# ubisoft/ubisoft-laforge-msmd

Hardware: AMD Instinct MI355X
Metric: FLAME frames/sec on 4s@16kHz clips (whole job; MSMD.forward motion-coefficient frames) (higher is better)
Workload: dtype bf16; 1 GPU; configs[1]: MSMD.forward, batch=32 x 4 s clips per GPU, wav2vec2-base encoder + 8-layer motion decoder, eval-mode, synthetic closed-form weights; batch_per_gpu=32, frames_per_clip=100, parallelism=dp1 (independent clips, no collective), launch=one hipGraph replay per step (the batch sits in the captured input buffers)

## Files before the change

### ubisoft-laforge-msmd_amd/csrc/gemm.hip

```cpp
#include "common.h"
#include <atomic>
#include <utility>

struct GemmArgs {
  const void* A; const void* W; const float* bias; const void* R; void* C;
  int M, N, K;
  long lda; int rows_per_batch; long a_batch_stride; long ldw, ldc, ldr;
  int act; int vec_ok; float inv_rpb;
  long strideA, strideW, strideC, strideBias, strideR;
  int mt, nt;
  int batch_inner; long strideA2, strideW2, strideC2;
  void* Z; float p_drop; const unsigned long* rng; unsigned site;
  int xn;
  int flags;
  const float* a_stats = nullptr; int a_nt = 0; const float* w_colsum = nullptr;
  const float* r_stats = nullptr; int r_nt = 0; const float* r_gamma = nullptr; const float* r_beta = nullptr;
  float* stats_out = nullptr; float ln_eps = 1e-5f;
  int stagger_ticks = 0;
};

enum : int {
  GF_WRITE_THROUGH = 1, GF_PAIRED_STORES = 2, GF_STAGGER = 4,
  GF_ACT_BWD = 8,
  GF_ONE_TILE = 16, GF_NO_256 = 32,
  GF_W_BELOW_32 = 64,
};
struct GemmActWord { int act, hint, flags; };
static constexpr GemmActWord gemm_unpack_act(int act) {
  return {act & 0xff, (act >> 8) & 0xff, ((act >> 16) & 7) | (((act >> 19) & 7) << 4)};
}
static_assert(gemm_unpack_act(MSMD_GEMM_WRITE_THROUGH).flags == GF_WRITE_THROUGH && gemm_unpack_act(MSMD_GEMM_PAIRED_STORES).flags == GF_PAIRED_STORES &&
              gemm_unpack_act(MSMD_GEMM_STAGGER).flags == GF_STAGGER && gemm_unpack_act(MSMD_GEMM_ONE_TILE_PER_WORKGROUP).flags == GF_ONE_TILE &&
              gemm_unpack_act(MSMD_GEMM_NO_256_TILE).flags == GF_NO_256 && gemm_unpack_act(MSMD_GEMM_W_BELOW_32).flags == GF_W_BELOW_32 && gemm_unpack_act(~0).flags == (0x7f & ~GF_ACT_BWD),
              "internal flag bits follow include/msmd_hip.h; no bit of `act` sets the internal one");
enum : int {
  GV_GENERIC = 0,
  GV_SPLIT_128 = 1, GV_SPLIT_64 = 5,
  GV_64_DEEP = 9, GV_64 = 12,
  GV_256x64 = 14,
  GV_192 = 15,
  GV_128 = 17,
  GV_128_AB = 13, GV_128_ONE_AB = 66,
  GV_256 = 80,
};

enum GemmEpi : int { EPI_ALL = 0, EPI_PLAIN = 1, EPI_LN_OPERAND = 2, EPI_LN_RESIDUAL = 3 };
constexpr int ACT_RUNTIME = -1;
constexpr int epia(GemmEpi e, int act) { return e + 10 * (1 + act); }
constexpr GemmEpi epia_family(int code) { return (GemmEpi)(code % 10); }
constexpr int epia_act(int code) { return code / 10 - 1; }

template <typename T> struct Mfma;
template <> struct Mfma<bf16_t> {
  static __device__ __forceinline__ void run(const u32x4& a, const u32x4& b, f32x4& acc) {
    acc = __builtin_amdgcn_mfma_f32_16x16x32_bf16(__builtin_bit_cast(bf16x8, a), __builtin_bit_cast(bf16x8, b),
                                                  acc, 0, 0, 0);
  }
};
template <> struct Mfma<f16_t> {
  static __device__ __forceinline__ void run(const u32x4& a, const u32x4& b, f32x4& acc) {
    acc = __builtin_amdgcn_mfma_f32_16x16x32_f16(__builtin_bit_cast(f16x8, a), __builtin_bit_cast(f16x8, b), acc, 0, 0, 0);
  }
};
template <> struct Mfma<float> {
  static __device__ __forceinline__ void run(const u32x4& a, const u32x4& b, f32x4& acc) {
#pragma unroll
    for (int e = 0; e < 4; ++e)
      acc = __builtin_amdgcn_mfma_f32_16x16x4f32(__uint_as_float(a[e]), __uint_as_float(b[e]), acc, 0, 0, 0);
  }
};

__device__ __forceinline__ int lds_off(int row, int chunk) { return row * 128 + ((chunk ^ ((row >> 1) & 7)) << 4); }

__device__ __forceinline__ long a_row_offset(const GemmArgs& p, int m) {
  if (p.rows_per_batch >= p.M) return (long)m * p.lda;
  int q = (int)((float)m * p.inv_rpb);
  int r = m - q * p.rows_per_batch;
  if (r < 0) { q -= 1; r += p.rows_per_batch; }
  if (r >= p.rows_per_batch) { q += 1; r -= p.rows_per_batch; }
  return (long)q * p.a_batch_stride + (long)r * p.lda;
}

template <typename TO> __device__ __forceinline__ float act_out(float x, int act) {
  if (act == MSMD_ACT_GELU) return sizeof(TO) == 2 ? gelu_poly16(x) : gelu_erf(x);
  if (act == MSMD_ACT_ELU) return elu1(x);
  return x;
}
template <typename TO, int ACT> __device__ __forceinline__ float act_out_c(float x, int act) {
  if constexpr (ACT == MSMD_ACT_GELU) return sizeof(TO) == 2 ? gelu_poly16(x) : gelu_erf(x);
  else if constexpr (ACT == MSMD_ACT_ELU) return elu1(x);
  else if constexpr (ACT == MSMD_ACT_NONE) return x;
  else return act_out<TO>(x, act);
}

__device__ __forceinline__ void store16_wt(void* p, const u32x4 v) {
  asm volatile("global_store_dwordx4 %0, %1, off sc1\n\ts_nop 1" ::"v"(p), "v"(v) : "memory");
}
__device__ __forceinline__ void store8_wt(void* p, const u32x2 v) {
  asm volatile("global_store_dwordx2 %0, %1, off sc1\n\ts_nop 1" ::"v"(p), "v"(v) : "memory");
}
template <typename TO> __device__ __forceinline__ void store4_out(TO* p, const float* v, bool wt) {
  if constexpr (sizeof(TO) == 4) {
    const f32x4 o = f32x4{v[0], v[1], v[2], v[3]};
    if (wt) store16_wt(p, __builtin_bit_cast(u32x4, o));
    else *(f32x4*)p = o;
  } else {
    const typename Vec4T<TO>::type o = pack4<TO>(v[0], v[1], v[2], v[3]);
    if (wt) store8_wt(p, __builtin_bit_cast(u32x2, o));
    else *(typename Vec4T<TO>::type*)p = o;
  }
}

template <typename TO, int FM, int FN, bool AB, bool LEAN, int ACT>
__device__ __forceinline__ void gemm_epilogue_interior(const GemmArgs& p, const f32x4 (&acc)[FN][FM], int z, int m_base,
                                                         int n_base, int fr, int fq) {
  TO* __restrict__ C = (TO*)p.C + (z / p.batch_inner) * p.strideC + (z % p.batch_inner) * p.strideC2 +
                       (long)(m_base + fr) * p.ldc + n_base + fq * 4;
  const TO* __restrict__ R = p.R ? (const TO*)p.R + z * p.strideR + (long)(m_base + fr) * p.ldr + n_base + fq * 4 : nullptr;
  const float* __restrict__ bias = p.bias ? p.bias + z * p.strideBias + n_base + fq * 4 : nullptr;
  const bool wt = p.flags & GF_WRITE_THROUGH;
  f32x4 bv[FN];
#pragma unroll
  for (int i = 0; i < FN; ++i) bv[i] = bias ? *(const f32x4*)(bias + i * 16) : f32x4{0.f, 0.f, 0.f, 0.f};
  typedef typename Vec4T<TO>::type V4;
// ... 100 lines not shown
#pragma unroll
      for (int e = 0; e < 4; ++e) v[e] = acc[i][j][e] + bv[e];
      TO* cp = C + (long)m * p.ldc + n;
      if (AB && (p.flags & GF_ACT_BWD)) {
        const TO* zp = (const TO*)p.Z + (cp - (TO*)p.C);
#pragma unroll
        for (int e = 0; e < 4; ++e)
          if (n + e < p.N) v[e] *= act_grad_fast((float)zp[e], ACT >= 0 ? ACT : p.act);
      } else {
        if (!LEAN && p.Z) {
          TO* zp = (TO*)p.Z + (cp - (TO*)p.C);
#pragma unroll
          for (int e = 0; e < 4; ++e)
            if (n + e < p.N) zp[e] = (TO)v[e];
        }
#pragma unroll
        for (int e = 0; e < 4; ++e) v[e] = act_out_c<TO, ACT>(v[e], p.act);
      }
      if (!LEAN && p.p_drop > 0.f) {
        const Philox4 rb = dropout_bits(p.rng, p.site, (unsigned long)(((long)m * p.N + n) >> 2));
        const unsigned thr = dropout_threshold(p.p_drop);
        const float c = 1.0f / (1.0f - p.p_drop);
        v[0] = rb.x >= thr ? v[0] * c : 0.f;
        v[1] = rb.y >= thr ? v[1] * c : 0.f;
        v[2] = rb.z >= thr ? v[2] * c : 0.f;
        v[3] = rb.w >= thr ? v[3] * c : 0.f;
      }
      if (p.vec_ok && n + 3 < p.N) {
        if (R) {
          const TO* rp = R + (long)m * p.ldr + n;
          if constexpr (sizeof(TO) == 4) {
            const f32x4 r = *(const f32x4*)rp;
#pragma unroll
            for (int e = 0; e < 4; ++e) v[e] += r[e];
          } else {
            const typename Vec4T<TO>::type r = *(const typename Vec4T<TO>::type*)rp;
#pragma unroll
            for (int e = 0; e < 4; ++e) v[e] += (float)r[e];
          }
        }
        store4_out<TO>(cp, v, p.flags & GF_WRITE_THROUGH);
      } else {
#pragma unroll
        for (int e = 0; e < 4; ++e) {
          if (n + e < p.N) {
            float o = v[e];
            if (R) o += to_f32(R[(long)m * p.ldr + n + e]);
            cp[e] = from_f32<TO>(o);
          }
        }
      }
    }
  }
}

template <int FM>
__device__ __forceinline__ void ln_issue(const float* stats, int nt, int M, int m_base, int fr, int fq, f32x2 (&raw)[FM][4]) {
#pragma unroll
  for (int j = 0; j < FM; ++j) {
    const f32x2* sp = (const f32x2*)stats + min(m_base + j * 16 + fr, M - 1);
#pragma unroll
    for (int q = 0; q < 4; ++q) raw[j][q] = fq + 4 * q < nt ? sp[(long)(fq + 4 * q) * M] : f32x2{0.f, 0.f};
  }
}

template <int FM>
__device__ __forceinline__ void ln_finish(const float* stats, int nt, int M, int m_base, int fr, int fq, const f32x2 (&raw)[FM][4],
                                          float inv_cols, float eps, float (&mu)[FM], float (&rs)[FM]) {
#pragma unroll
  for (int j = 0; j < FM; ++j) {
    float S = (raw[j][0][0] + raw[j][1][0]) + (raw[j][2][0] + raw[j][3][0]);
    float Q = (raw[j][0][1] + raw[j][1][1]) + (raw[j][2][1] + raw[j][3][1]);
    if (nt > 16) {
      const f32x2* sp = (const f32x2*)stats + min(m_base + j * 16 + fr, M - 1);
      for (int t = 16 + fq; t < nt; t += 4) { const f32x2 w = sp[(long)t * M]; S += w[0]; Q += w[1]; }
    }
    S += __shfl_xor(S, 16, 64); S += __shfl_xor(S, 32, 64);
    Q += __shfl_xor(Q, 16, 64); Q += __shfl_xor(Q, 32, 64);
    mu[j] = S * inv_cols;
    rs[j] = rsqrtf(fmaxf(Q * inv_cols - mu[j] * mu[j], 0.f) + eps);
  }
}

template <typename TO, int FM, int FN, int MODE, int ACT = -1>
__device__ __forceinline__ void gemm_epilogue_ln(const GemmArgs& p, const f32x4 (&acc)[FN][FM], int m_base, int n_base,
                                                 int fr, int fq, const f32x2 (&raw)[FM][4]) {
  static_assert((FN == 4 || FN == 2) && (FM >= 2 && FM <= 4), "one wave = one statistics slab of 16 FN columns, 2 to 4 fragment rows");
  constexpr int SLAB = FN * 16;
  constexpr int IB = FM == 3 ? 2 : FN;
  typedef typename Vec4T<TO>::type V4;
  const int n = n_base + fq * 4;
  float mu[FM], rs[FM];
#pragma unroll
  for (int j = 0; j < FM; ++j) { mu[j] = 0.f; rs[j] = 1.f; }
  if constexpr (MODE == 1) ln_finish<FM>(p.a_stats, p.a_nt, p.M, m_base, fr, fq, raw, 1.0f / (float)p.K, p.ln_eps, mu, rs);
  else if (p.r_stats) ln_finish<FM>(p.r_stats, p.r_nt, p.M, m_base, fr, fq, raw, 1.0f / (float)p.N, p.ln_eps, mu, rs);
  float rowS[FM], rowQ[FM], tS[FM], tQ[FM], prS[FM], prQ[FM];
#pragma unroll
  for (int j = 0; j < FM; ++j) rowS[j] = rowQ[j] = tS[j] = tQ[j] = prS[j] = prQ[j] = 0.f;
  const bool odd = fq & 1;
  const bool pair = sizeof(TO) == 2 && (p.flags & GF_PAIRED_STORES);
#pragma unroll
  for (int i0 = 0; i0 < FN; i0 += IB) {
    f32x4 bv[IB], xv[IB], yv[IB];
    V4 rr[FM][IB];
#pragma unroll
    for (int ii = 0; ii < IB; ++ii) bv[ii] = *(const f32x4*)(p.bias + n + (i0 + ii) * 16);
    if constexpr (MODE == 1) {
#pragma unroll
      for (int ii = 0; ii < IB; ++ii) xv[ii] = *(const f32x4*)(p.w_colsum + n + (i0 + ii) * 16);
    } else {
#pragma unroll
      for (int j = 0; j < FM; ++j) {
        const TO* rp = (const TO*)p.R + (long)min(m_base + j * 16 + fr, p.M - 1) * p.ldr + n;
#pragma unroll
        for (int ii = 0; ii < IB; ++ii) rr[j][ii] = *(const V4*)(rp + (i0 + ii) * 16);
      }
      if (p.r_stats) {
#pragma unroll
        for (int ii = 0; ii < IB; ++ii) { xv[ii] = *(const f32x4*)(p.r_gamma + n + (i0 + ii) * 16); yv[ii] = *(const f32x4*)(p.r_beta + n + (i0 + ii) * 16); }
      } else {
#pragma unroll
        for (int ii = 0; ii < IB; ++ii) { xv[ii] = f32x4{1.f, 1.f, 1.f, 1.f}; yv[ii] = f32x4{0.f, 0.f, 0.f, 0.f}; }
      }
    }
#pragma unroll
    for (int ii = 0; ii < IB; ++ii) {
      const int i = i0 + ii;
      V4 o[FM];
#pragma unroll
      for (int j = 0; j < FM; ++j) {
        float v[4];
#pragma unroll
        for (int e = 0; e < 4; ++e) {
          float x = acc[i][j][e];
          if constexpr (MODE == 1) x = rs[j] * (x - mu[j] * xv[ii][e]);
          v[e] = act_out_c<TO, ACT>(x + bv[ii][e], p.act);
          if constexpr (MODE == 2) v[e] += fmaf(((float)rr[j][ii][e] - mu[j]) * rs[j], xv[ii][e], yv[ii][e]);
        }
        if constexpr (sizeof(TO) == 4) o[j] = V4{v[0], v[1], v[2], v[3]};
        else o[j] = pack4<TO>(v[0], v[1], v[2], v[3]);
        if constexpr (MODE == 2) {
          float pS = 0.f, pQ = 0.f;
#pragma unroll
          for (int e = 0; e < 4; ++e) { const float w = (float)o[j][e]; pS += w; pQ = fmaf(w, w, pQ); }
          if ((i & 1) == 0) { tS[j] = pS; tQ[j] = pQ; }
          else {
            const float aS = tS[j] + pS, aQ = tQ[j] + pQ;
            if (FN == 2) { rowS[j] = aS; rowQ[j] = aQ; }
            else if ((i & 2) == 0) { prS[j] = aS; prQ[j] = aQ; }
            else { rowS[j] = prS[j] + aS; rowQ[j] = prQ[j] + aQ; }
          }
        }
      }
      bool stored = false;
      if constexpr (sizeof(TO) == 2) {
        if (pair) {
#pragma unroll
          for (int jp = 0; jp + 1 < FM; jp += 2) {
            const u32x2 a = __builtin_bit_cast(u32x2, o[jp]), b = __builtin_bit_cast(u32x2, o[jp + 1]);
            const u32x2 send = odd ? a : b;
            u32x2 recv;
            recv[0] = __shfl_xor(send[0], 16, 64);
            recv[1] = __shfl_xor(send[1], 16, 64);
            const u32x4 w = odd ? u32x4{recv[0], recv[1], b[0], b[1]} : u32x4{a[0], a[1], recv[0], recv[1]};
            const int m = m_base + jp * 16 + (odd ? 16 : 0) + fr;
            if (m < p.M) *(u32x4*)((TO*)p.C + (long)m * p.ldc + n + i * 16 - (odd ? 4 : 0)) = w;
          }
          if constexpr (FM % 2 == 1) {
            const int m2 = m_base + (FM - 1) * 16 + fr;
            if (m2 < p.M) *(V4*)((TO*)p.C + (long)m2 * p.ldc + n + i * 16) = o[FM - 1];
          }
          stored = true;
        }
      }
      if (!stored) {
#pragma unroll
        for (int j = 0; j < FM; ++j) {
          const int m = m_base + j * 16 + fr;
          if (m < p.M) *(V4*)((TO*)p.C + (long)m * p.ldc + n + i * 16) = o[j];
        }
      }
    }
  }
  if constexpr (MODE == 2) {
    if (p.stats_out) {
#pragma unroll
      for (int j = 0; j < FM; ++j) {
        rowS[j] += __shfl_xor(rowS[j], 16, 64); rowS[j] += __shfl_xor(rowS[j], 32, 64);
        rowQ[j] += __shfl_xor(rowQ[j], 16, 64); rowQ[j] += __shfl_xor(rowQ[j], 32, 64);
        const int m = m_base + j * 16 + fr;
        if (fq == 0 && m < p.M) *(f32x2*)(p.stats_out + ((long)(n_base / SLAB) * p.M + m) * 2) = f32x2{rowS[j], rowQ[j]};
      }
    }
  }
}

template <typename T, typename TO, int BM, int BN>
__global__ __launch_bounds__(256) void gemm_kernel(const GemmArgs p) {
  constexpr int E = 16 / sizeof(T);
  constexpr int BKE = 128 / sizeof(T);
  constexpr int LA = BM / 32, LW = BN / 32;
  constexpr int FM = BM / 32, FN = BN / 32;
  __shared__ __attribute__((aligned(16))) unsigned char smem[2 * (BM + BN) * 128];

  const int pid = blockIdx.x;
// ... 57 lines not shown
  const int nk = (p.K + BKE - 1) / BKE;
  load_global(0);
  store_lds(0);
  __syncthreads();
  for (int kt = 0; kt < nk; ++kt) {
    const int cur = kt & 1;
    if (kt + 1 < nk) load_global((kt + 1) * BKE);
    const unsigned char* sa = smem + cur * (BM + BN) * 128;
    const unsigned char* sw = sa + BM * 128;
#pragma unroll
    for (int g = 0; g < 2; ++g) {
      u32x4 fx[FM], fw[FN];
#pragma unroll
      for (int j = 0; j < FM; ++j) fx[j] = *(const u32x4*)(sa + lds_off(wm + j * 16 + fr, g * 4 + fq));
#pragma unroll
      for (int i = 0; i < FN; ++i) fw[i] = *(const u32x4*)(sw + lds_off(wn + i * 16 + fr, g * 4 + fq));
#pragma unroll
      for (int i = 0; i < FN; ++i)
#pragma unroll
        for (int j = 0; j < FM; ++j) Mfma<T>::run(fw[i], fx[j], acc[i][j]);
    }
    if (kt + 1 < nk) store_lds(cur ^ 1);
    __syncthreads();
  }

  gemm_epilogue<TO, FM, FN>(p, acc, z, m0 + wm, n0 + wn, fr, fq);
}

typedef __attribute__((address_space(3))) void lds_void_t;
typedef __attribute__((address_space(1))) const void gbl_void_t;

template <typename TO, int BM, int BN, int WM, int WN, int NSTAGE, bool PIPE = false, typename TI = bf16_t, int EPIA = 0>
__global__ __launch_bounds__(WM * WN * 64, (WM * WN == 8 && NSTAGE * (BM + BN) * 128 <= 80 * 1024 && (epia_family(EPIA) != EPI_ALL || BM * BN <= 128 * 128)) ? 4 : 1) void gemm2_kernel(const GemmArgs p) {
  constexpr int EPI = epia_family(EPIA), ACTK = epia_act(EPIA);
  constexpr int NW = WM * WN, NT = NW * 64;
  constexpr int STAGE = (BM + BN) * 128;
  constexpr int LPT = (BM + BN) * 8 / NT;
  constexpr int FM = BM / WM / 16, FN = BN / WN / 16;
  static_assert((BM + BN) * 8 % NT == 0, "tile chunks must divide over the threads");
  extern __shared__ __attribute__((aligned(16))) unsigned char smem[];

  const int pid = blockIdx.x;
  const int xcd = pid & 7, slot = pid >> 3;
  const int xm_n = 8 / p.xn, ntx = (p.nt + p.xn - 1) / p.xn;
  const int m_tile = (slot / ntx) * xm_n + (xcd % xm_n), n_tile = (slot % ntx) * p.xn + xcd / xm_n;
  if (m_tile >= p.mt || n_tile >= p.nt) return;
  const int z = blockIdx.z;
  const int zo = z / p.batch_inner, zi = z % p.batch_inner;
  const bf16_t* __restrict__ A = (const bf16_t*)p.A + zo * p.strideA + zi * p.strideA2;
  const bf16_t* __restrict__ W = (const bf16_t*)p.W + zo * p.strideW + zi * p.strideW2;
  const int m0 = m_tile * BM, n0 = n_tile * BN;
  const int tid = threadIdx.x, lane = tid & 63, wid = tid >> 6;

  const bf16_t* src[LPT];
#pragma unroll
  for (int i = 0; i < LPT; ++i) {
    const int id = (i * NW + wid) * 64 + lane;
    const int row = id >> 3, phys = id & 7;
    const int c = phys ^ ((row >> 1) & 7);
    if (row < BM) {
      const int m = min(m0 + row, p.M - 1);
      src[i] = A + a_row_offset(p, m) + c * 8;
    } else {
      const int n = min(n0 + row - BM, p.N - 1);
      src[i] = W + (long)n * p.ldw + c * 8;
    }
  }
  auto issue = [&](int kt, int stage) {
#pragma unroll
    for (int i = 0; i < LPT; ++i)
      __builtin_amdgcn_global_load_lds((gbl_void_t*)(src[i] + kt * 64),
                                       (lds_void_t*)(smem + stage * STAGE + (i * NW + wid) * 1024), 16, 0, 0);
  };

  const int wm = (wid / WN) * (BM / WM), wn = (wid % WN) * (BN / WN);
  const int fr = lane & 15, fq = lane >> 4;
  f32x4 acc[FN][FM];
#pragma unroll
  for (int i = 0; i < FN; ++i)
#pragma unroll
    for (int j = 0; j < FM; ++j) acc[i][j] = f32x4{0.f, 0.f, 0.f, 0.f};

  const int nk = p.K / 64;
#pragma unroll
  for (int s = 0; s < NSTAGE - 1; ++s)
    if (s < nk) issue(s, s);
  if (p.stagger_ticks > 0 && ((pid >> 8) & 1) && pid < 512) {
    const unsigned long t0 = __builtin_amdgcn_s_memrealtime();
    while ((long)(__builtin_amdgcn_s_memrealtime() - t0) < p.stagger_ticks) __builtin_amdgcn_s_sleep(16);
  }
  constexpr bool LNK = (BN == 128 || BN == 64) && WN == 2 && (FM == 2 || FM == 3) && sizeof(TO) == 2;
  constexpr bool LN_LATE = FM == 3;
  f32x2 lnraw[(LNK && !LN_LATE) ? FM : 1][4];
  if constexpr (LNK && !LN_LATE && EPI != 1) {
    if (EPI == 2 || (EPI == 0 && p.a_stats)) ln_issue<FM>(p.a_stats, p.a_nt, p.M, m0 + wm, fr, fq, lnraw);
    else if (p.r_stats) ln_issue<FM>(p.r_stats, p.r_nt, p.M, m0 + wm, fr, fq, lnraw);
  }
  int stage = 0;
  for (int kt = 0; kt < nk; ++kt) {
    if (kt + NSTAGE - 2 < nk) asm volatile("s_waitcnt vmcnt(%0)" ::"n"((NSTAGE - 2) * LPT) : "memory");
    else asm volatile("s_waitcnt vmcnt(0)" ::: "memory");
    __builtin_amdgcn_s_barrier();
    if (kt + NSTAGE - 1 < nk) issue(kt + NSTAGE - 1, (stage + NSTAGE - 1) % NSTAGE);
    const unsigned char* sa = smem + stage * STAGE;
    const unsigned char* sw = sa + BM * 128;
    if constexpr (PIPE) {
      u32x4 fx[2][FM], fw[2][FN];
#pragma unroll
      for (int g = 0; g < 2; ++g) {
#pragma unroll
        for (int j = 0; j < FM; ++j) fx[g][j] = *(const u32x4*)(sa + lds_off(wm + j * 16 + fr, g * 4 + fq));
#pragma unroll
        for (int i = 0; i < FN; ++i) fw[g][i] = *(const u32x4*)(sw + lds_off(wn + i * 16 + fr, g * 4 + fq));
      }
      __builtin_amdgcn_sched_barrier(0);
#pragma unroll
      for (int g = 0; g < 2; ++g) {
#pragma unroll
        for (int i = 0; i < FN; ++i)
#pragma unroll
          for (int j = 0; j < FM; ++j) Mfma<TI>::run(fw[g][i], fx[g][j], acc[i][j]);
        __builtin_amdgcn_sched_barrier(0);
      }
    } else {
#pragma unroll
      for (int g = 0; g < 2; ++g) {
        u32x4 fx[FM], fw[FN];
#pragma unroll
        for (int j = 0; j < FM; ++j) fx[j] = *(const u32x4*)(sa + lds_off(wm + j * 16 + fr, g * 4 + fq));
#pragma unroll
        for (int i = 0; i < FN; ++i) fw[i] = *(const u32x4*)(sw + lds_off(wn + i * 16 + fr, g * 4 + fq));
#pragma unroll
        for (int i = 0; i < FN; ++i)
#pragma unroll
          for (int j = 0; j < FM; ++j) Mfma<TI>::run(fw[i], fx[j], acc[i][j]);
      }
    }
    stage = (stage + 1 == NSTAGE) ? 0 : stage + 1;
  }
  int tid_e = tid;
  if constexpr (LN_LATE) asm volatile("" : "+v"(tid_e));
  const int wm_e = ((tid_e >> 6) / WN) * (BM / WM), wn_e = ((tid_e >> 6) % WN) * (BN / WN);
  const int fr_e = tid_e & 15, fq_e = (tid_e & 63) >> 4;
  auto run_epilogue = [&]() {
    if constexpr (EPI == 1) { gemm_epilogue<TO, FM, FN, false, true, ACTK>(p, acc, z, m0 + wm_e, n0 + wn_e, fr_e, fq_e); return; }
    if constexpr (LNK && !LN_LATE && EPI == 2) { gemm_epilogue_ln<TO, FM, FN, 1, ACTK>(p, acc, m0 + wm_e, n0 + wn_e, fr_e, fq_e, lnraw); return; }
    if constexpr (LNK && !LN_LATE && EPI == 3) { gemm_epilogue_ln<TO, FM, FN, 2, ACTK>(p, acc, m0 + wm_e, n0 + wn_e, fr_e, fq_e, lnraw); return; }
    if constexpr (LNK && LN_LATE && (EPI == 2 || EPI == 3)) {
      f32x2 late[FM][4];
      if constexpr (EPI == 2) ln_issue<FM>(p.a_stats, p.a_nt, p.M, m0 + wm_e, fr_e, fq_e, late);
      else if (p.r_stats) ln_issue<FM>(p.r_stats, p.r_nt, p.M, m0 + wm_e, fr_e, fq_e, late);
      gemm_epilogue_ln<TO, FM, FN, EPI - 1, ACTK>(p, acc, m0 + wm_e, n0 + wn_e, fr_e, fq_e, late);
      return;
    }
    if constexpr (LNK && !LN_LATE) {
      if (p.a_stats) { gemm_epilogue_ln<TO, FM, FN, 1, ACTK>(p, acc, m0 + wm_e, n0 + wn_e, fr_e, fq_e, lnraw); return; }
      if (p.r_stats || p.stats_out) { gemm_epilogue_ln<TO, FM, FN, 2, ACTK>(p, acc, m0 + wm_e, n0 + wn_e, fr_e, fq_e, lnraw); return; }
    }
    if constexpr (LNK && LN_LATE) {
      if (p.a_stats || p.r_stats || p.stats_out) {
        f32x2 late[FM][4];
        if (p.a_stats) ln_issue<FM>(p.a_stats, p.a_nt, p.M, m0 + wm_e, fr_e, fq_e, late);
        else if (p.r_stats) ln_issue<FM>(p.r_stats, p.r_nt, p.M, m0 + wm_e, fr_e, fq_e, late);
        if (p.a_stats) gemm_epilogue_ln<TO, FM, FN, 1, ACTK>(p, acc, m0 + wm_e, n0 + wn_e, fr_e, fq_e, late);
        else gemm_epilogue_ln<TO, FM, FN, 2, ACTK>(p, acc, m0 + wm_e, n0 + wn_e, fr_e, fq_e, late);
        return;
      }
    }
    gemm_epilogue<TO, FM, FN, sizeof(TO) == 2, false, ACTK>(p, acc, z, m0 + wm_e, n0 + wn_e, fr_e, fq_e);
  };
  run_epilogue();
}

template <typename TO, int BM, int BN, int WM, int WN, typename TI, int EPIA>
__global__ __launch_bounds__(WM * WN * 64, 4) void gemm2p_kernel(const GemmArgs p) {
  constexpr int EPI = epia_family(EPIA), ACTK = epia_act(EPIA);
  constexpr int NW = WM * WN, NT = NW * 64;
  constexpr int STAGE = (BM + BN) * 128;
  constexpr int LPT = (BM + BN) * 8 / NT;
  constexpr int FM = BM / WM / 16, FN = BN / WN / 16;
  static_assert(EPI >= 1 && EPI <= 3 && sizeof(TO) == 2 && NW == 8 && WN == 2 && BN == 128 && (FM == 2 || FM == 3), "the hot 8-wave tiles, inference epilogues");
  static_assert((BM + BN) * 8 % NT == 0, "tile chunks must divide over the threads");
  constexpr bool LN_LATE = FM == 3;
  extern __shared__ __attribute__((aligned(16))) unsigned char smem[];
  const int tid = threadIdx.x;
  const int xm_n = 8 / p.xn, ntx = (p.nt + p.xn - 1) / p.xn;
  const int vgrid = ((p.mt + xm_n - 1) / xm_n) * ntx * 8;
  const TI* __restrict__ A = (const TI*)p.A;
  const TI* __restrict__ W = (const TI*)p.W;
  auto next_tile = [&](int vb, int& m0, int& n0) -> int {
    for (; vb < vgrid; vb += gridDim.x) {
      const int xcd = vb & 7, slot = vb >> 3;
      const int m_tile = (slot / ntx) * xm_n + (xcd % xm_n), n_tile = (slot % ntx) * p.xn + xcd / xm_n;
      if (m_tile < p.mt && n_tile < p.nt) { m0 = m_tile * BM; n0 = n_tile * BN; return vb; }
    }
    return -1;
  };
  const TI* src[LPT];
  auto set_src = [&](int m0, int n0, int t) {
    const int lane = t & 63, wid = t >> 6;
#pragma unroll
    for (int i = 0; i < LPT; ++i) {
      const int id = (i * NW + wid) * 64 + lane;
      const int row = id >> 3, phys = id & 7;
      const int c = phys ^ ((row >> 1) & 7);
      if (row < BM) src[i] = A + a_row_offset(p, min(m0 + row, p.M - 1)) + c * 8;
      else src[i] = W + (long)min(n0 + row - BM, p.N - 1) * p.ldw + c * 8;
    }
  };
  auto issue = [&](int kt, int stage, int t) {
    const int wid = t >> 6;
#pragma unroll
    for (int i = 0; i < LPT; ++i)
      __builtin_amdgcn_global_load_lds((gbl_void_t*)(src[i] + kt * 64),
                                       (lds_void_t*)(smem + stage * STAGE + (i * NW + wid) * 1024), 16, 0, 0);
  };
  int m0 = 0, n0 = 0;
  int vb = next_tile(blockIdx.x, m0, n0);
  if (vb < 0) return;
  const int nk = p.K / 64;
  set_src(m0, n0, tid);
  int stage = 0;
  issue(0, 0, tid);
  for (;;) {
    int t_k = tid;
    asm volatile("" : "+v"(t_k));
    const int wm = ((t_k >> 6) / WN) * (BM / WM), wn = ((t_k >> 6) % WN) * (BN / WN);
    const int fr = t_k & 15, fq = (t_k & 63) >> 4;
    f32x2 lnraw[LN_LATE ? 1 : FM][4];
// ... 749 lines not shown
  if (p.Z || p.p_drop > 0.f || (p.flags & GF_ACT_BWD)) return false;
  if (((uintptr_t)p.bias & 15) || ((uintptr_t)p.C & 7) || ((uintptr_t)p.R & 7)) return false;
  if ((gemm_last_row_offset(p) + p.K) * 2 >= (1L << 32) || ((long)(p.N - 1) * p.ldw + p.K) * 2 >= (1L << 32)) return false;
  const GemmEpi epi = epia_family(gemm_epia(p, true));
  if ((p.a_stats || p.r_stats) && ((p.M & 1) || ((uintptr_t)p.a_stats & 15) || ((uintptr_t)p.r_stats & 15))) return false;
  if (epi == EPI_LN_OPERAND && (p.R || !p.bias || !p.w_colsum)) return false;
  if (epi == EPI_LN_RESIDUAL && (!p.R || !p.bias || p.act != MSMD_ACT_NONE)) return false;
  return p.act == MSMD_ACT_NONE || p.act == MSMD_ACT_GELU;
}

static bool gemm8_wins(int M, int N, int K) {
  const long tiles = (long)((M + 255) / 256) * (N / 256);
  if (tiles < 192) return false;
  const double fill = (double)tiles / (256.0 * (double)((tiles + 255) / 256));
  return fill >= 0.75 && (K >= 1024 || fill >= 0.878);
}

constexpr int GEMM8_RING = 2 * 4 * 128 * 128;
template <auto KFN, int LDS>
static int launch_gemm8(GemmArgs& p, hipStream_t st) {
  p.mt = (p.M + 255) / 256; p.nt = p.N / 256;
  const int tiles = p.mt * p.nt, cap = gemm8_workgroup_cap();
  if (tiles <= 512) p.flags |= GF_WRITE_THROUGH;
  return gemm_launch_kernel<KFN>(dim3(tiles < cap ? tiles : cap), 512, LDS, st, p);
}

static bool gemm8s_takes(const GemmArgs& p, int batch, bool split_out) {
  if (batch != 1 || p.batch_inner != 1 || (p.N % 256) || (p.K % 32) || p.K < 64 || !p.vec_ok) return false;
  if (((uintptr_t)p.bias & 15) || ((uintptr_t)p.C & 15) || ((uintptr_t)p.R & 15)) return false;
  if (split_out ? ((p.ldc % 32) || (p.R && (p.ldr % 32))) : ((p.ldc % 4) || (p.R && (p.ldr % 4)))) return false;
  if ((gemm_last_row_offset(p) + 2L * p.K) * 2 >= (1L << 32) || ((long)(p.N - 1) * p.ldw + 2L * p.K) * 2 >= (1L << 32)) return false;
  return p.act == MSMD_ACT_NONE || p.act == MSMD_ACT_GELU;
}
static bool gemm8s_wins(int M, int N, int K, bool w_below_32) {
  const long tiles = (long)((M + 255) / 256) * (N / 256);
  if (tiles < 160) return false;
  const double fill = (double)tiles / (256.0 * (double)((tiles + 255) / 256));
  return fill >= (w_below_32 ? 0.65 : 0.75);
}

template <typename TO, int BM, int BN, int WM, int WN, int NSTAGE>
static int launch_gemm2s(GemmArgs& p, int batch, hipStream_t st) {
  constexpr int lds = NSTAGE * (BM + BN) * 128;
  const dim3 grid(gemm2_xcd_grid(p, BM, BN, p.lda / 2), 1, batch);
  return dispatch_code<0, 1>((p.flags & GF_W_BELOW_32) != 0, [&](auto ws) {
    auto run = [&](auto act) {
      return gemm_launch_kernel<gemm2s_kernel<TO, BM, BN, WM, WN, NSTAGE, decltype(act)::value, decltype(ws)::value != 0>>(grid, WM * WN * 64, lds, st, p);
    };
    int r = -1;
    if constexpr (lds <= 80 * 1024) r = dispatch_code<MSMD_ACT_NONE, MSMD_ACT_GELU>(p.act, run);
    return r >= 0 ? r : run(std::integral_constant<int, ACT_RUNTIME>{});
  });
}

template <typename TO>
static int dispatch_gemm2s(GemmArgs& p, int batch, hipStream_t st, int variant) {
  switch (variant) {
    case GV_SPLIT_128: return launch_gemm2s<TO, 128, 128, 4, 2, 2>(p, batch, st);
    case GV_SPLIT_64: return launch_gemm2s<TO, 64, 64, 2, 2, 4>(p, batch, st);
    case GV_256x64: return launch_gemm2s<TO, 256, 64, 8, 1, 2>(p, batch, st);
    case GV_256:
      if (!gemm8s_takes(p, batch, sizeof(TO) == 2)) return -1;
      return dispatch_code<11, 21>(epia(EPI_PLAIN, p.act), [&](auto c) {
        return dispatch_code<0, 1>((p.flags & GF_W_BELOW_32) != 0, [&](auto ws) {
          return launch_gemm8<gemm8_kernel<f16_t, decltype(c)::value, (sizeof(TO) == 4 ? 2 : 1) + 4 * decltype(ws)::value>, GEMM8_RING>(p, st);
        });
      });
    default: return -1;
  }
}

template <typename T, typename TO>
static int launch_gemm(GemmArgs& p, int batch, hipStream_t st) {
  const bool small = (p.N <= 64) || ((long)((p.M + 127) / 128) * ((p.N + 127) / 128) * batch < 128);
  const int B = small ? 64 : 128;
  p.mt = (p.M + B - 1) / B; p.nt = (p.N + B - 1) / B;
  const dim3 grid(((p.mt + 7) / 8) * 8 * p.nt, 1, batch);
  return small ? gemm_launch_kernel<gemm_kernel<T, TO, 64, 64>>(grid, 256, 0, st, p)
               : gemm_launch_kernel<gemm_kernel<T, TO, 128, 128>>(grid, 256, 0, st, p);
}

static constexpr bool gemm2_has(int variant, bool bf16) {
  if (variant == GV_128_AB || variant == GV_128_ONE_AB) return bf16;
  return variant == GV_64_DEEP || variant == GV_64 || variant == GV_256x64 || variant == GV_192 || variant == GV_128 || variant == GV_256;
}

template <typename TO, typename TI>
static int dispatch_gemm(GemmArgs& p, int batch, hipStream_t st, int variant) {
  if (variant == GV_GENERIC) return launch_gemm<TI, TO>(p, batch, st);
  if constexpr (sizeof(TI) == 2) {
    if (!gemm2_has(variant, __is_same(TI, bf16_t))) return -1;
    if constexpr (__is_same(TI, bf16_t)) {
      if (variant == GV_128_AB) return launch_gemm2<TO, 128, 128, 4, 2, 2>(p, gemm2_xcd_grid(p, 128, 128, p.lda), batch, st);
      if (variant == GV_128_ONE_AB) return launch_gemm2<TO, 128, 128, 4, 2, 2, true>(p, gemm2_xcd_grid(p, 128, 128, p.lda), batch, st);
    }
    switch (variant) {
      case GV_64_DEEP: return launch_gemm2_epi<TO, 64, 64, 2, 2, 4, false, TI>(p, batch, st);
      case GV_64: return launch_gemm2_epi<TO, 64, 64, 2, 2, 2, false, TI>(p, batch, st);
      case GV_256x64: return launch_gemm2_epi<TO, 256, 64, 8, 1, 2, true, TI>(p, batch, st);
      case GV_192: return launch_gemm2_epi<TO, 192, 128, 4, 2, 2, true, TI>(p, batch, st);
      case GV_128: return launch_gemm2_epi<TO, 128, 128, 4, 2, 2, true, TI>(p, batch, st);
    }
    if constexpr (sizeof(TO) == 2) {
      if (!gemm8_takes(p, batch, 2)) return -1;
      return dispatch_code<11, 21, 12, 22, 13>(gemm_epia(p, true), [&](auto c) {
        constexpr int E = decltype(c)::value;
        return launch_gemm8<gemm8_kernel<TI, E>, GEMM8_RING + (epia_family(E) >= EPI_LN_OPERAND ? 8 * 4096 : 0)>(p, st);
      });
    }
  }
  return -1;
}

static bool tall_rounds_favour_192(int M, long tiles128, long tiles192) {
  if (M < 9600 || tiles192 < 256) return false;
  const double fill128 = (double)tiles128 / (512.0 * (double)((tiles128 + 511) / 512));
  const double fill192 = (double)tiles192 / (512.0 * (double)((tiles192 + 511) / 512));
  return 1.2 * fill192 > 1.03 * fill128;
}

struct GemmCall {
  const void* A = nullptr; const void* W = nullptr; const float* bias = nullptr; const void* residual = nullptr; void* C = nullptr;
  int M = 0, N = 0, K = 0, in_dtype = 0, out_dtype = 0;
  long lda = 0; int rows_per_batch = 0; long a_batch_stride = 0; long ldw = 0, ldc = 0, ldr = 0;
  int act = 0;
  int batch = 1; long strideA = 0, strideW = 0, strideC = 0, strideBias = 0, strideR = 0;
  int batch_inner = 1; long strideA2 = 0, strideW2 = 0, strideC2 = 0;
  void* z_out = nullptr; float p_drop = 0.f; const unsigned long* rng = nullptr; unsigned site = 0; int internal_flags = 0;
  const float* a_stats = nullptr; const float* w_colsum = nullptr; const float* r_stats = nullptr; const float* r_gamma = nullptr; const float* r_beta = nullptr;
  float* stats_out = nullptr; int slab_in = 0, slab_out = 0; float eps = 1e-5f;
};

static GemmArgs gemm_args(const GemmCall& c, int act, int flags, int osz, int ab = 1) {
  GemmArgs p{};
  const int rows_per_batch = c.rows_per_batch <= 0 ? c.M : c.rows_per_batch;
  p.A = c.A; p.W = c.W; p.bias = c.bias; p.R = c.residual; p.C = c.C;
  p.M = c.M; p.N = c.N; p.K = c.K;
  p.lda = ab * c.lda; p.rows_per_batch = rows_per_batch; p.a_batch_stride = ab * c.a_batch_stride;
  p.ldw = ab * c.ldw; p.ldc = c.ldc; p.ldr = c.ldr; p.act = act;
  p.inv_rpb = 1.0f / (float)rows_per_batch;
  p.strideA = ab * c.strideA; p.strideW = ab * c.strideW; p.strideC = c.strideC; p.strideBias = c.strideBias; p.strideR = c.strideR;
  p.batch_inner = c.batch_inner; p.strideA2 = ab * c.strideA2; p.strideW2 = ab * c.strideW2; p.strideC2 = c.strideC2;
  p.xn = 1;
  p.vec_ok = osz == 0 ||
             ((c.ldc % 4 == 0) && (c.strideC % 4 == 0) && (c.strideC2 % 4 == 0) && (((uintptr_t)c.C % (4 * osz)) == 0) &&
              (!c.residual || ((c.ldr % 4 == 0) && (c.strideR % 4 == 0) && (((uintptr_t)c.residual % (4 * osz)) == 0))));
  if ((flags & GF_PAIRED_STORES) && (osz != 2 || (c.ldc % 8) || (c.strideC % 8) || (c.strideC2 % 8) || ((uintptr_t)c.C % 16) || !p.vec_ok))
    flags &= ~GF_PAIRED_STORES;
  p.flags = flags;
  return p;
}

static int gemm_split_route(const GemmArgs& p, int nz, bool split_out, int hint, int flags) {
  const bool takes8 = gemm8s_takes(p, nz, split_out);
  if (hint == GV_256 && !takes8) hint = 0;
  if (hint) return (hint == GV_SPLIT_128 || hint == GV_SPLIT_64 || hint == GV_256x64 || hint == GV_256) ? hint : -1;
  if (!(flags & GF_NO_256) && (flags & GF_W_BELOW_32) && takes8 && gemm8s_wins(p.M, p.N, p.K, true)) return GV_256;
  if (p.N <= 64) return (long)((p.M + 255) / 256) * nz >= 256 ? GV_256x64 : GV_SPLIT_64;
  return (long)((p.M + 127) / 128) * ((p.N + 127) / 128) * nz >= 192 ? GV_SPLIT_128 : GV_SPLIT_64;
}

static int gemm16_route(const GemmArgs& p, int nz, int osz, bool bf16, int hint, int flags, int cols = 0) {
  const bool takes8 = (cols != 64 || !p.stats_out) && gemm8_takes(p, nz, osz);
  const bool rule8 = hint == 0 && !(flags & GF_NO_256);
  if (!(hint == GV_256 ? takes8 : !cols || (cols == 128 && (hint == GV_192 || hint == GV_128 || hint == GV_128_ONE_AB)))) hint = 0;
  if (hint) return gemm2_has(hint, bf16) ? hint : GV_GENERIC;
  const int M = p.M, N = p.N;
  const long tiles128 = (long)((M + 127) / 128) * ((N + 127) / 128) * nz;
  const long tiles192 = (long)((M + 191) / 192) * ((N + 127) / 128) * nz;
  const bool wide = cols ? cols == 128 : N > 64;
  if (rule8 && takes8 && gemm8_wins(M, N, p.K)) return GV_256;
  if (wide && M >= 16000 && tiles192 >= 400) return GV_192;
  if (wide && osz == 2 && !p.Z && !(p.p_drop > 0.f) && !(p.flags & GF_ACT_BWD) && tall_rounds_favour_192(M, tiles128, tiles192)) return GV_192;
  if (cols ? wide : wide && tiles128 >= 192) return GV_128;
  if (!cols && N <= 64 && (long)((M + 255) / 256) * nz >= 256) return GV_256x64;
  return p.K >= 1024 ? GV_64_DEEP : GV_64;
}

static int gemm_plan(GemmArgs& p, const GemmCall& c) {
  if (c.M <= 0 || c.N <= 0 || c.K <= 0 || c.batch <= 0 || c.batch_inner <= 0 || !c.A || !c.W || !c.C) return -1;
  const GemmActWord u = gemm_unpack_act(c.act);
  const int flags = u.flags | c.internal_flags, nz = c.batch * c.batch_inner;
  const auto strides_divide = [&](int E) {
    return !(c.K % E || c.lda % E || c.ldw % E || c.a_batch_stride % E || c.strideA % E || c.strideW % E || c.strideA2 % E || c.strideW2 % E);
  };
  if (c.in_dtype == MSMD_F16X2) {
    if (c.out_dtype != MSMD_F32 && c.out_dtype != MSMD_F16X2) return -1;
    if (!strides_divide(32) || c.z_out || c.p_drop != 0.f) return -1;
    if (((uintptr_t)c.A & 15) || ((uintptr_t)c.W & 15) || ((uintptr_t)c.C & 15)) return -1;
    if (c.out_dtype == MSMD_F16X2) {
      if ((c.N & 3) || c.ldc % 32 || c.strideC % 32 || c.strideC2 % 32 || (c.residual && (c.ldr % 32 || c.strideR % 32))) return -1;
      if (c.bias && (((uintptr_t)c.bias & 15) || (c.strideBias & 3))) return -1;
    }
    p = gemm_args(c, u.act, flags & (GF_WRITE_THROUGH | GF_W_BELOW_32), c.out_dtype == MSMD_F32 ? 4 : 0, 2);
    return gemm_split_route(p, nz, c.out_dtype == MSMD_F16X2, u.hint, flags);
  }
  if (c.in_dtype == MSMD_F32 ? (c.out_dtype != MSMD_F32 && c.out_dtype != MSMD_F16 && c.out_dtype != MSMD_BF16)
                             : ((c.in_dtype != MSMD_F16 && c.in_dtype != MSMD_BF16) || (c.out_dtype != c.in_dtype && c.out_dtype != MSMD_F32)))
    return -1;
  if (!strides_divide(c.in_dtype == MSMD_F32 ? 4 : 8)) return -1;
  if (((uintptr_t)c.A & 15) || ((uintptr_t)c.W & 15)) return -1;
  if (c.p_drop != 0.f && (!(c.p_drop > 0.f && c.p_drop < 1.f) || !c.rng || (c.N & 3) || c.ldc != c.N || c.batch != 1 || c.batch_inner != 1))
    return -1;
  const int osz = c.out_dtype == MSMD_F32 ? 4 : 2;
  p = gemm_args(c, u.act, flags, osz);
  p.Z = c.z_out; p.p_drop = c.p_drop; p.rng = c.rng; p.site = c.site;
  if (c.in_dtype == MSMD_F32 || (c.K % 64)) return GV_GENERIC;
  return gemm16_route(p, nz, osz, c.in_dtype == MSMD_BF16, u.hint, flags);
}

static int gemm_launch(GemmArgs& p, int in_dtype, int out_dtype, int nz, int variant, hipStream_t st) {
  switch (in_dtype * 4 + out_dtype) {
    case MSMD_F16X2 * 4 + MSMD_F32: return dispatch_gemm2s<float>(p, nz, st, variant);
    case MSMD_F16X2 * 4 + MSMD_F16X2: return dispatch_gemm2s<f16_t>(p, nz, st, variant);
    case MSMD_BF16 * 4 + MSMD_BF16: return dispatch_gemm<bf16_t, bf16_t>(p, nz, st, variant);
    case MSMD_BF16 * 4 + MSMD_F32: return dispatch_gemm<float, bf16_t>(p, nz, st, variant);
    case MSMD_F16 * 4 + MSMD_F16: return dispatch_gemm<f16_t, f16_t>(p, nz, st, variant);
    case MSMD_F16 * 4 + MSMD_F32: return dispatch_gemm<float, f16_t>(p, nz, st, variant);
    case MSMD_F32 * 4 + MSMD_F32: return dispatch_gemm<float, float>(p, nz, st, variant);
    case MSMD_F32 * 4 + MSMD_F16: return dispatch_gemm<f16_t, float>(p, nz, st, variant);
    case MSMD_F32 * 4 + MSMD_BF16: return dispatch_gemm<bf16_t, float>(p, nz, st, variant);
  }
  return -1;
}

static int gemm_run(int (*plan)(GemmArgs&, const GemmCall&), const GemmCall& c, msmd_stream_t stream) {
  GemmArgs p;
  const int variant = plan(p, c);
  const int r = variant < 0 ? -1 : gemm_launch(p, c.in_dtype, c.out_dtype, c.batch * c.batch_inner, variant, (hipStream_t)stream);
  return r >= 0 ? r : 1;
}

static GemmCall gemm_ex_call(const void* A, const void* W, const float* bias, const void* residual, void* C, int M, int N, int K, int in_dtype,
                             int out_dtype, long lda, int rows_per_batch, long a_batch_stride, long ldw, long ldc, long ldr, int act, int batch,
                             long strideA, long strideW, long strideC, long strideBias, long strideR, void* z_out, float p_drop,
                             const unsigned long* rng_state, unsigned int site) {
  GemmCall c;
  c.A = A; c.W = W; c.bias = bias; c.residual = residual; c.C = C;
  c.M = M; c.N = N; c.K = K; c.in_dtype = in_dtype; c.out_dtype = out_dtype;
  c.lda = lda; c.rows_per_batch = rows_per_batch; c.a_batch_stride = a_batch_stride; c.ldw = ldw; c.ldc = ldc; c.ldr = ldr;
  c.act = act; c.batch = batch;
  c.strideA = strideA; c.strideW = strideW; c.strideC = strideC; c.strideBias = strideBias; c.strideR = strideR;
  c.z_out = z_out; c.p_drop = p_drop; c.rng = rng_state; c.site = site;
  return c;
}

extern "C" int msmd_gemm_ex(const void* A, const void* W, const float* bias, const void* residual, void* C, int M, int N, int K, int in_dtype,
                            int out_dtype, long lda, int rows_per_batch, long a_batch_stride, long ldw, long ldc, long ldr, int act, int batch,
                            long strideA, long strideW, long strideC, long strideBias, long strideR, void* z_out, float p_drop,
                            const unsigned long* rng_state, unsigned int site, msmd_stream_t stream) {
  return gemm_run(gemm_plan, gemm_ex_call(A, W, bias, residual, C, M, N, K, in_dtype, out_dtype, lda, rows_per_batch, a_batch_stride, ldw, ldc, ldr,
                                          act, batch, strideA, strideW, strideC, strideBias, strideR, z_out, p_drop, rng_state, site), stream);
}

extern "C" int msmd_gemm(const void* A, const void* W, const float* bias, const void* residual, void* C, int M, int N, int K, int in_dtype,
                         int out_dtype, long lda, int rows_per_batch, long a_batch_stride, long ldw, long ldc, long ldr, int act, int batch,
// ... 91 lines not shown
```

Before: 829,400 frames/s.

## Add 64x128 GEMM tile variant with early-issued LayerNorm-residual epilogue operands

Adds a 64x128 tile variant (4 waves) to the generic GEMM and routes mid-size LN-column GEMMs to it when the 128x128 grid would leave most compute units idle. For the LayerNorm-residual epilogue on this tile, the residual, bias, gamma/beta and row statistics loads are issued before the K loop so their latency overlaps the main loop. The cost is extra registers held across the mainloop, which may lower occupancy.

```diff
diff --git a/ubisoft-laforge-msmd_amd/csrc/gemm.hip b/ubisoft-laforge-msmd_amd/csrc/gemm.hip
--- a/ubisoft-laforge-msmd_amd/csrc/gemm.hip
+++ b/ubisoft-laforge-msmd_amd/csrc/gemm.hip
@@ -40,6 +40,7 @@
   GV_256x64 = 14,
   GV_192 = 15,
   GV_128 = 17,
+  GV_64x128 = 18,
   GV_128_AB = 13, GV_128_ONE_AB = 66,
   GV_256 = 80,
 };
@@ -306,9 +307,31 @@
   }
 }
 
-template <typename TO, int FM, int FN, int MODE, int ACT = -1>
+template <typename TO, int FM, int FN> struct LnResOps { f32x4 bv[FN], xv[FN], yv[FN]; typename Vec4T<TO>::type rr[FM][FN]; };
+template <typename TO, int FM, int FN>
+__device__ __forceinline__ void ln_res_issue(const GemmArgs& p, int m_base, int n_base, int fr, int fq, LnResOps<TO, FM, FN>& o) {
+  typedef typename Vec4T<TO>::type V4;
+  const int n = n_base + fq * 4;
+#pragma unroll
+  for (int i = 0; i < FN; ++i) o.bv[i] = *(const f32x4*)(p.bias + n + i * 16);
+#pragma unroll
+  for (int j = 0; j < FM; ++j) {
+    const TO* rp = (const TO*)p.R + (long)min(m_base + j * 16 + fr, p.M - 1) * p.ldr + n;
+#pragma unroll
+    for (int i = 0; i < FN; ++i) o.rr[j][i] = *(const V4*)(rp + i * 16);
+  }
+  if (p.r_stats) {
+#pragma unroll
+    for (int i = 0; i < FN; ++i) { o.xv[i] = *(const f32x4*)(p.r_gamma + n + i * 16); o.yv[i] = *(const f32x4*)(p.r_beta + n + i * 16); }
+  } else {
+#pragma unroll
+    for (int i = 0; i < FN; ++i) { o.xv[i] = f32x4{1.f, 1.f, 1.f, 1.f}; o.yv[i] = f32x4{0.f, 0.f, 0.f, 0.f}; }
+  }
+}
+
+template <typename TO, int FM, int FN, int MODE, int ACT = -1, bool EARLY = false>
 __device__ __forceinline__ void gemm_epilogue_ln(const GemmArgs& p, const f32x4 (&acc)[FN][FM], int m_base, int n_base,
-                                                 int fr, int fq, const f32x2 (&raw)[FM][4]) {
+                                                 int fr, int fq, const f32x2 (&raw)[FM][4], const LnResOps<TO, FM, FN>* early = nullptr) {
   static_assert((FN == 4 || FN == 2) && (FM >= 2 && FM <= 4), "one wave = one statistics slab of 16 FN columns, 2 to 4 fragment rows");
   constexpr int SLAB = FN * 16;
   constexpr int IB = FM == 3 ? 2 : FN;
@@ -328,24 +351,34 @@
   for (int i0 = 0; i0 < FN; i0 += IB) {
     f32x4 bv[IB], xv[IB], yv[IB];
     V4 rr[FM][IB];
-#pragma unroll
-    for (int ii = 0; ii < IB; ++ii) bv[ii] = *(const f32x4*)(p.bias + n + (i0 + ii) * 16);
-    if constexpr (MODE == 1) {
-#pragma unroll
-      for (int ii = 0; ii < IB; ++ii) xv[ii] = *(const f32x4*)(p.w_colsum + n + (i0 + ii) * 16);
+    if constexpr (EARLY) {
+      static_assert(MODE == 2 && IB == FN, "the early operands are the LayerNorm-residual form's, all fragment columns at once");
+#pragma unroll
+      for (int ii = 0; ii < IB; ++ii) {
+        bv[ii] = early->bv[ii]; xv[ii] = early->xv[ii]; yv[ii] = early->yv[ii];
+#pragma unroll
+        for (int j = 0; j < FM; ++j) rr[j][ii] = early->rr[j][ii];
+      }
     } else {
 #pragma unroll
-      for (int j = 0; j < FM; ++j) {
-        const TO* rp = (const TO*)p.R + (long)min(m_base + j * 16 + fr, p.M - 1) * p.ldr + n;
-#pragma unroll
-        for (int ii = 0; ii < IB; ++ii) rr[j][ii] = *(const V4*)(rp + (i0 + ii) * 16);
-      }
-      if (p.r_stats) {
-#pragma unroll
-        for (int ii = 0; ii < IB; ++ii) { xv[ii] = *(const f32x4*)(p.r_gamma + n + (i0 + ii) * 16); yv[ii] = *(const f32x4*)(p.r_beta + n + (i0 + ii) * 16); }
+      for (int ii = 0; ii < IB; ++ii) bv[ii] = *(const f32x4*)(p.bias + n + (i0 + ii) * 16);
+      if constexpr (MODE == 1) {
+#pragma unroll
+        for (int ii = 0; ii < IB; ++ii) xv[ii] = *(const f32x4*)(p.w_colsum + n + (i0 + ii) * 16);
       } else {
 #pragma unroll
-        for (int ii = 0; ii < IB; ++ii) { xv[ii] = f32x4{1.f, 1.f, 1.f, 1.f}; yv[ii] = f32x4{0.f, 0.f, 0.f, 0.f}; }
+        for (int j = 0; j < FM; ++j) {
+          const TO* rp = (const TO*)p.R + (long)min(m_base + j * 16 + fr, p.M - 1) * p.ldr + n;
+#pragma unroll
+          for (int ii = 0; ii < IB; ++ii) rr[j][ii] = *(const V4*)(rp + (i0 + ii) * 16);
+        }
+        if (p.r_stats) {
+#pragma unroll
+          for (int ii = 0; ii < IB; ++ii) { xv[ii] = *(const f32x4*)(p.r_gamma + n + (i0 + ii) * 16); yv[ii] = *(const f32x4*)(p.r_beta + n + (i0 + ii) * 16); }
+        } else {
+#pragma unroll
+          for (int ii = 0; ii < IB; ++ii) { xv[ii] = f32x4{1.f, 1.f, 1.f, 1.f}; yv[ii] = f32x4{0.f, 0.f, 0.f, 0.f}; }
+        }
       }
     }
 #pragma unroll
@@ -569,6 +602,16 @@
     for (int j = 0; j < FM; ++j) acc[i][j] = f32x4{0.f, 0.f, 0.f, 0.f};
 
   const int nk = p.K / 64;
+  constexpr bool LNK = (BN == 128 || BN == 64) && WN == 2 && (FM == 2 || FM == 3) && sizeof(TO) == 2;
+  constexpr bool LN_LATE = FM == 3;
+  constexpr bool EARLY_OPS = LNK && EPI == 3 && NW == 4 && BM == 64 && BN == 128;
+  f32x2 lnraw[(LNK && !LN_LATE) ? FM : 1][4];
+  std::conditional_t<EARLY_OPS, LnResOps<TO, FM, FN>, char> early;
+  (void)early;
+  if constexpr (EARLY_OPS) {
+    if (p.r_stats) ln_issue<FM>(p.r_stats, p.r_nt, p.M, m0 + wm, fr, fq, lnraw);
+    ln_res_issue<TO, FM, FN>(p, m0 + wm, n0 + wn, fr, fq, early);
+  }
 #pragma unroll
   for (int s = 0; s < NSTAGE - 1; ++s)
     if (s < nk) issue(s, s);
@@ -576,10 +619,7 @@
     const unsigned long t0 = __builtin_amdgcn_s_memrealtime();
     while ((long)(__builtin_amdgcn_s_memrealtime() - t0) < p.stagger_ticks) __builtin_amdgcn_s_sleep(16);
   }
-  constexpr bool LNK = (BN == 128 || BN == 64) && WN == 2 && (FM == 2 || FM == 3) && sizeof(TO) == 2;
-  constexpr bool LN_LATE = FM == 3;
-  f32x2 lnraw[(LNK && !LN_LATE) ? FM : 1][4];
-  if constexpr (LNK && !LN_LATE && EPI != 1) {
+  if constexpr (LNK && !LN_LATE && EPI != 1 && !EARLY_OPS) {
     if (EPI == 2 || (EPI == 0 && p.a_stats)) ln_issue<FM>(p.a_stats, p.a_nt, p.M, m0 + wm, fr, fq, lnraw);
     else if (p.r_stats) ln_issue<FM>(p.r_stats, p.r_nt, p.M, m0 + wm, fr, fq, lnraw);
   }
@@ -632,6 +672,7 @@
   auto run_epilogue = [&]() {
     if constexpr (EPI == 1) { gemm_epilogue<TO, FM, FN, false, true, ACTK>(p, acc, z, m0 + wm_e, n0 + wn_e, fr_e, fq_e); return; }
     if constexpr (LNK && !LN_LATE && EPI == 2) { gemm_epilogue_ln<TO, FM, FN, 1, ACTK>(p, acc, m0 + wm_e, n0 + wn_e, fr_e, fq_e, lnraw); return; }
+    if constexpr (EARLY_OPS) { gemm_epilogue_ln<TO, FM, FN, 2, ACTK, true>(p, acc, m0 + wm_e, n0 + wn_e, fr_e, fq_e, lnraw, &early); return; }
     if constexpr (LNK && !LN_LATE && EPI == 3) { gemm_epilogue_ln<TO, FM, FN, 2, ACTK>(p, acc, m0 + wm_e, n0 + wn_e, fr_e, fq_e, lnraw); return; }
     if constexpr (LNK && LN_LATE && (EPI == 2 || EPI == 3)) {
       f32x2 late[FM][4];
@@ -1547,7 +1588,7 @@
 
 static constexpr bool gemm2_has(int variant, bool bf16) {
   if (variant == GV_128_AB || variant == GV_128_ONE_AB) return bf16;
-  return variant == GV_64_DEEP || variant == GV_64 || variant == GV_256x64 || variant == GV_192 || variant == GV_128 || variant == GV_256;
+  return variant == GV_64_DEEP || variant == GV_64 || variant == GV_256x64 || variant == GV_192 || variant == GV_128 || variant == GV_64x128 || variant == GV_256;
 }
 
 template <typename TO, typename TI>
@@ -1565,6 +1606,7 @@
       case GV_256x64: return launch_gemm2_epi<TO, 256, 64, 8, 1, 2, true, TI>(p, batch, st);
       case GV_192: return launch_gemm2_epi<TO, 192, 128, 4, 2, 2, true, TI>(p, batch, st);
       case GV_128: return launch_gemm2_epi<TO, 128, 128, 4, 2, 2, true, TI>(p, batch, st);
+      case GV_64x128: return launch_gemm2_epi<TO, 64, 128, 2, 2, 4, true, TI>(p, batch, st);
     }
     if constexpr (sizeof(TO) == 2) {
       if (!gemm8_takes(p, batch, 2)) return -1;
@@ -1628,7 +1670,7 @@
 static int gemm16_route(const GemmArgs& p, int nz, int osz, bool bf16, int hint, int flags, int cols = 0) {
   const bool takes8 = (cols != 64 || !p.stats_out) && gemm8_takes(p, nz, osz);
   const bool rule8 = hint == 0 && !(flags & GF_NO_256);
-  if (!(hint == GV_256 ? takes8 : !cols || (cols == 128 && (hint == GV_192 || hint == GV_128 || hint == GV_128_ONE_AB)))) hint = 0;
+  if (!(hint == GV_256 ? takes8 : !cols || (cols == 128 && (hint == GV_192 || hint == GV_128 || hint == GV_128_ONE_AB || hint == GV_64x128)))) hint = 0;
   if (hint) return gemm2_has(hint, bf16) ? hint : GV_GENERIC;
   const int M = p.M, N = p.N;
   const long tiles128 = (long)((M + 127) / 128) * ((N + 127) / 128) * nz;
@@ -1637,6 +1679,8 @@
   if (rule8 && takes8 && gemm8_wins(M, N, p.K)) return GV_256;
   if (wide && M >= 16000 && tiles192 >= 400) return GV_192;
   if (wide && osz == 2 && !p.Z && !(p.p_drop > 0.f) && !(p.flags & GF_ACT_BWD) && tall_rounds_favour_192(M, tiles128, tiles192)) return GV_192;
+  const long tiles64x128 = (long)((M + 63) / 64) * ((N + 127) / 128) * nz;
+  if (cols == 128 && osz == 2 && !p.Z && !(p.p_drop > 0.f) && !(p.flags & GF_ACT_BWD) && tiles128 >= 32 && tiles64x128 <= 256) return GV_64x128;
   if (cols ? wide : wide && tiles128 >= 192) return GV_128;
   if (!cols && N <= 64 && (long)((M + 255) / 256) * nz >= 256) return GV_256x64;
   return p.K >= 1024 ? GV_64_DEEP : GV_64;
```

Result: faster. 856,000 frames/s, median of 6 (+3.2%).
